# ZhenghaoFei/visual_odom

Hardware: AMD Instinct MI355X
Metric: stereo frames/sec on KITTI-00 1241x376 @ ~2000 features (higher is better)
Workload: dtype u8/int32 LK (f32 2x2 solve), f64 pose solve

## Files before the change

visual_odom_amd/csrc/lk.hip:

```cpp
#include "vo_kernels.h"
#include "vo_lkmath.h"

#include <float.h>

namespace vo {

constexpr int LK_WIN = 21;
constexpr int LK_JT_W = 48, LK_JT_H = 40;
constexpr int LK_W_BITS = 14;

struct __attribute__((packed, aligned(1))) LkU2 {
    uint32_t lo, hi;
};
struct __attribute__((packed, aligned(4))) LkU4 {
    uint32_t a, b, c, d;
};

__device__ __forceinline__ void lk_weights(float a, float b, uint32_t &wt, uint32_t &wb)
{
    const float s = (float)(1 << LK_W_BITS), magic = 12582912.f;
    const float a1 = (1.f - a) * s, a0 = a * s, b1 = 1.f - b;
    const uint32_t r00 = (uint32_t)__float_as_int(a1 * b1 + magic);
    const uint32_t r01 = (uint32_t)__float_as_int(a0 * b1 + magic);
    const uint32_t r10 = (uint32_t)__float_as_int(a1 * b + magic);
    const uint32_t iw11 = ((1u << LK_W_BITS) + 3u * 0x4B400000u) - (r00 + r01 + r10);
    wt = perm_b32(r01, r00, VO_SEL_LO16);
    wb = perm_b32(iw11, r10, VO_SEL_LO16);
}

#ifndef VO_LK_ATTRS
#define VO_LK_ATTRS __launch_bounds__(64, 7)
#endif
template <bool SPLIT>
__device__ __forceinline__ void lk_circular_body(const PyrImage *__restrict__ imgs, const Quad *__restrict__ quads,
                                                 const float2 *__restrict__ pts_in, const int *__restrict__ n_pts, int cap,
                                                 int n_frames, int fpg , int ppp ,
                                                 float2 *__restrict__ trk,
                                                 uint8_t *__restrict__ status,
                                                 const LkParams prm, int hop_begin, int hop_end)
{
    __shared__ __attribute__((aligned(16))) uint8_t s_jt[LK_JT_H * LK_JT_W];

    const int bid = blockIdx.x;
    const int xcd = bid & 7, slot = bid >> 3;
    const int grp = slot / ppp, fi = slot - grp * ppp;
    const int frame = grp * fpg + (xcd & (fpg - 1));
    const int f = (xcd / fpg) * ppp + fi;
    if (frame >= n_frames || f >= n_pts[frame])
        return;
    const int lane = threadIdx.x;
    const bool live = lane < 63;
    const int lr = live ? lane : 62;
    const int r = lr / 3, c0 = 7 * (lr - 3 * r);
    const int lane_off = r * LK_JT_W + c0;

    const Quad q = quads[frame];
    const float halfWin = (LK_WIN - 1) * 0.5f;
    const float FLT_SCALE = 1.f / (1 << 20);
    const float eps_lo = (float)(prm.epsilon * 0.999999), eps_hi = (float)(prm.epsilon * 1.000001);
    const float min_eig_n = prm.min_eig * (1.001f * (float)(2 * LK_WIN * LK_WIN));

    const float2 p = pts_in[(size_t)frame * cap + f];
    float prevPtX = unif(p.x), prevPtY = unif(p.y);
    if (SPLIT && hop_begin > 0) {
        const size_t o = ((size_t)frame * 4 + (hop_begin - 1)) * cap + f;
        const float2 q0 = trk[o];
        const bool dead0 = status[o] == 0 || q0.x < 0.f || q0.y < 0.f || (hop_begin == 1 && (p.x < 0.f || p.y < 0.f));
        if (dead0 && !prm.full_chain)
            return;
        prevPtX = unif(q0.x);
        prevPtY = unif(q0.y);
    }

    for (int hop = SPLIT ? hop_begin : 0; hop < (SPLIT ? hop_end : 4); hop++) {
        const int pi = hop == 0 ? q.l0 : hop == 1 ? q.r0 : hop == 2 ? q.r1 : q.l1;
        const int ni = hop == 0 ? q.r0 : hop == 1 ? q.r1 : hop == 2 ? q.l1 : q.l0;
        const PyrImage &I = imgs[pi];
        const PyrImage &J = imgs[ni];
        float outX = 0.f, outY = 0.f;
        int st = 1;

        for (int level = prm.max_level; level >= 0; level--) {
            const float scale = __int_as_float((127 - level) << 23);
            float prevX = prevPtX * scale, prevY = prevPtY * scale;
            float nextX, nextY;
            if (level == prm.max_level) {
                nextX = prevX;
                nextY = prevY;
            } else {
                nextX = outX * 2.f;
                nextY = outY * 2.f;
            }
            outX = nextX;
            outY = nextY;

            const int iw = I.w[level], ih = I.h[level], istride = I.stride[level];
            const int jw = J.w[level], jh = J.h[level], jstride = J.stride[level];
            const VO_GLOBAL uint8_t *__restrict__ Iimg = (const VO_GLOBAL uint8_t *)I.lvl[level];
            const VO_GLOBAL uint32_t *__restrict__ Ider = (const VO_GLOBAL uint32_t *)I.der[level];
            const VO_GLOBAL uint8_t *__restrict__ Jimg = (const VO_GLOBAL uint8_t *)J.lvl[level];

            prevX -= halfWin;
            prevY -= halfWin;
            const float fpx = floorf(prevX), fpy = floorf(prevY);
            const int ipx = uni(vo_f2i(fpx)), ipy = uni(vo_f2i(fpy));
            if (VO_BALLOT(__builtin_isunordered(fpx, fpy)) != 0ull || ipx < -LK_WIN || ipx >= iw || ipy < -LK_WIN || ipy >= ih) {
                if (level == 0)
                    st = 0;
                continue;
            }
            uint32_t wt, wb;
            lk_weights(prevX - fpx, prevY - fpy, wt, wb);

            uint32_t Ixp[4], Iyp[4];
            int a11 = 0, a12 = 0, a22 = 0, c1 = 0, c2 = 0;
            {
                const ptrdiff_t org = (ptrdiff_t)VO_BY * istride + VO_BX;
                const VO_GLOBAL uint8_t *Ib = Iimg - org;
                const VO_GLOBAL uint8_t *Db = (const VO_GLOBAL uint8_t *)(Ider - org);
                const uint32_t o = (uint32_t)((ipy + r + VO_BY) * istride + ipx + c0 + VO_BX);
                const uint32_t od = live ? 4u * o : 0u, drow = 4u * (uint32_t)istride;
                const LkU2 t = *(const VO_GLOBAL LkU2 *)(Ib + o);
                const LkU2 u = *(const VO_GLOBAL LkU2 *)(Ib + (o + (uint32_t)istride));
                const LkU4 dt0 = *(const VO_GLOBAL LkU4 *)(Db + od);
                const LkU4 dt1 = *(const VO_GLOBAL LkU4 *)(Db + (od + 16u));
                const LkU4 db0 = *(const VO_GLOBAL LkU4 *)(Db + (od + drow));
                const LkU4 db1 = *(const VO_GLOBAL LkU4 *)(Db + (od + drow + 16u));
                const uint32_t dt[8] = {dt0.a, dt0.b, dt0.c, dt0.d, dt1.a, dt1.b, dt1.c, dt1.d};
                const uint32_t db[8] = {db0.a, db0.b, db0.c, db0.d, db1.a, db1.b, db1.c, db1.d};
                uint32_t Ip[4];
                bilinear7_u8(t.lo, t.hi, u.lo, u.hi, wt, wb, Ip);
                bilinear7_deriv(dt, db, wt, wb, Ixp, Iyp);
                a11 = sdot2_first(Ixp[0], Ixp[0], 0);
                a12 = sdot2_first(Ixp[0], Iyp[0], 0);
                a22 = sdot2_first(Iyp[0], Iyp[0], 0);
                c1 = sdot2_first(Ip[0], Ixp[0], 0);
                c2 = sdot2_first(Ip[0], Iyp[0], 0);
#pragma unroll
                for (int m = 1; m < 4; m++) {
                    a11 = sdot2(Ixp[m], Ixp[m], a11);
                    a12 = sdot2(Ixp[m], Iyp[m], a12);
                    a22 = sdot2(Iyp[m], Iyp[m], a22);
                    c1 = sdot2(Ip[m], Ixp[m], c1);
                    c2 = sdot2(Ip[m], Iyp[m], c2);
                }
            }
            float A11, A12, A22;
            wave_sum3_exact_f32(a11, a12, a22, A11, A12, A22);
            A11 *= FLT_SCALE;
            A12 *= FLT_SCALE;
            A22 *= FLT_SCALE;

            float D = A11 * A22 - A12 * A12;
            const float t = A22 + A11;
            const float s2 = (A11 - A22) * (A11 - A22) + 4.f * A12 * A12;
            const float u = t - (min_eig_n + t * 3.814697265625e-6f);
            bool eig_ok = u > 0.f && s2 < u * u * 0.9999f;
            if (__builtin_expect(!eig_ok, 0)) {
#ifndef VO_HOST_EMUL
                asm volatile("" ::: "memory");
#endif
                const float minEig = (t - sqrtf(s2)) / (float)(2 * LK_WIN * LK_WIN);
                eig_ok = !(minEig < prm.min_eig);
            }
            if (!eig_ok || D < FLT_EPSILON) {
                if (level == 0)
                    st = 0;
                continue;
            }
            D = 1.f / D;
            const float A11s = A11 * FLT_SCALE, A12s = A12 * FLT_SCALE, A22s = A22 * FLT_SCALE;
            const int nc1 = -c1, nc2 = -c2;

            nextX -= halfWin;
            nextY -= halfWin;
            float prevDX = 0.f, prevDY = 0.f;
            int jx0 = 0, jy0 = 0;
            bool have_tile = false;
            static_assert(LK_JT_W % 16 == 0 && VO_BX % 4 == 0, "16-byte tile chunks at 4-byte aligned origins");
            static_assert(VO_BY >= LK_WIN && LK_JT_W >= LK_WIN + 1 + 12 + 3 && LK_JT_H >= LK_WIN + 1 + 9,
                          "a tile clamped to the row end / the last border row still covers the window of every corner the "
                          "reference admits (up to w - 1, h - 1: the borders are at least a window wide)");
            const int jx_max = jstride - VO_BX - LK_JT_W, jy_max = jh + VO_BY - LK_JT_H;

            int j = 0;
            float fnx = floorf(nextX), fny = floorf(nextY);
            bool run = prm.max_count > 0;
            while (run) {
                const int inx = uni(vo_f2i(fnx)), iny = uni(vo_f2i(fny));
                if (VO_BALLOT(__builtin_isunordered(fnx, fny)) != 0ull || inx < -LK_WIN || inx >= jw || iny < -LK_WIN || iny >= jh) {
                    if (level == 0)
                        st = 0;
                    break;
                }
                if (!have_tile || inx < jx0 || inx + LK_WIN + 1 > jx0 + LK_JT_W || iny < jy0 ||
                    iny + LK_WIN + 1 > jy0 + LK_JT_H) {
                    jx0 = (inx - 12) & ~3;
                    jy0 = iny - 9;
                    jx0 = jx0 < -VO_BX ? -VO_BX : jx0 > jx_max ? jx_max : jx0;
                    jy0 = jy0 < -VO_BY ? -VO_BY : jy0 > jy_max ? jy_max : jy0;
                    __syncthreads();
                    const VO_GLOBAL uint8_t *tb = Jimg + (ptrdiff_t)jy0 * jstride + jx0;
                    for (int c = lane; c < LK_JT_H * (LK_JT_W / 16); c += 64) {
                        const int row = c / (LK_JT_W / 16), col = c - row * (LK_JT_W / 16);
                        const LkU4 v = *(const VO_GLOBAL LkU4 *)(tb + (uint32_t)(row * jstride + 16 * col));
                        *reinterpret_cast<uint4 *>(&s_jt[row * LK_JT_W + 16 * col]) = make_uint4(v.a, v.b, v.c, v.d);
                    }
                    __syncthreads();
                    have_tile = true;
                }
                uint32_t Jt[7], Jb[7];
                {
                    const int off = (iny - jy0) * LK_JT_W + (inx - jx0) + lane_off;
                    const LkU2 t = *reinterpret_cast<const LkU2 *>(&s_jt[off]);
                    const LkU2 u = *reinterpret_cast<const LkU2 *>(&s_jt[off + LK_JT_W]);
                    lift7(t.lo, t.hi, Jt);
                    lift7(u.lo, u.hi, Jb);
                }
                for (;;) {
                    lk_weights(nextX - fnx, nextY - fny, wt, wb);
                    int b1, b2;
                    {
                        uint32_t Jp[4];
                        blend7(Jt, Jb, wt, wb, Jp);
                        b1 = sdot2_first(Jp[0], Ixp[0], nc1);
                        b2 = sdot2_first(Jp[0], Iyp[0], nc2);
#pragma unroll
                        for (int m = 1; m < 4; m++) {
                            b1 = sdot2(Jp[m], Ixp[m], b1);
                            b2 = sdot2(Jp[m], Iyp[m], b2);
                        }
                    }
                    float fb1, fb2;
                    wave_sum2_exact_f32(b1, b2, fb1, fb2);
                    const float dx = (A12s * fb2 - A22s * fb1) * D;
                    const float dy = (A12s * fb1 - A11s * fb2) * D;
                    nextX += dx;
                    nextY += dy;
                    outX = nextX + halfWin;
                    outY = nextY + halfWin;
                    const float n2 = fmaf(dy, dy, dx * dx);
                    if (__builtin_expect(!(n2 > eps_hi), 0)) {
#ifndef VO_HOST_EMUL
                        asm volatile("" ::: "memory");
#endif
                        if (n2 < eps_lo || (double)dx * dx + (double)dy * dy <= prm.epsilon) {
                            run = false;
                            break;
                        }
                    }
                    if (j > 0 && fabsf(dx + prevDX) <= 0.01f && fabsf(dy + prevDY) <= 0.01f) {
#ifndef VO_HOST_EMUL
                        asm volatile("" ::: "memory");
#endif
                        outX -= dx * 0.5f;
                        outY -= dy * 0.5f;
                        run = false;
                        break;
                    }
                    prevDX = dx;
                    prevDY = dy;
                    if (++j >= prm.max_count) {
                        run = false;
                        break;
                    }
                    const uint32_t ua = (uint32_t)__float_as_int(nextX - fnx), ub = (uint32_t)__float_as_int(nextY - fny);
                    if (VO_BALLOT((ua > ub ? ua : ub) >= 0x3f800000u) != 0ull) {
                        fnx = floorf(nextX);
                        fny = floorf(nextY);
                        break;
                    }
                }
            }

            if (st && level == 0) {
                const int fx = vo_f2i(floorf(outX - halfWin)), fy = vo_f2i(floorf(outY - halfWin));
                if (fx < -LK_WIN || fx >= jw || fy < -LK_WIN || fy >= jh)
                    st = 0;
            }
        }

        if (lane == 0) {
            trk[((size_t)frame * 4 + hop) * cap + f] = make_float2(outX, outY);
            status[((size_t)frame * 4 + hop) * cap + f] = (uint8_t)st;
        }
        const bool dead = st == 0 || outX < 0.f || outY < 0.f || (hop == 0 && (p.x < 0.f || p.y < 0.f));
        if (dead && !prm.full_chain && hop < 3) {
            if (lane == 0)
                for (int k = hop + 1; k < 4; k++) {
                    trk[((size_t)frame * 4 + k) * cap + f] = make_float2(-1.f, -1.f);
                    status[((size_t)frame * 4 + k) * cap + f] = 0;
                }
            return;
        }
        prevPtX = unif(outX);
        prevPtY = unif(outY);
    }
}

__global__ VO_LK_ATTRS void lk_circular_kernel(const PyrImage *__restrict__ imgs,
                                                          const Quad *__restrict__ quads,
                                                          const float2 *__restrict__ pts_in,
                                                          const int *__restrict__ n_pts, int cap,
                                                          int n_frames, int fpg ,
                                                          int ppp ,
                                                          float2 *__restrict__ trk,
                                                          uint8_t *__restrict__ status,
                                                          LkParams prm)
{
    lk_circular_body<false>(imgs, quads, pts_in, n_pts, cap, n_frames, fpg, ppp, trk, status, prm, 0, 4);
}

__global__ VO_LK_ATTRS void lk_hops_kernel(const PyrImage *__restrict__ imgs, const Quad *__restrict__ quads,
                                           const float2 *__restrict__ pts_in, const int *__restrict__ n_pts, int cap,
                                           int n_frames, int fpg, int ppp, float2 *__restrict__ trk,
                                           uint8_t *__restrict__ status, LkParams prm, int hop_begin, int hop_end)
{
    lk_circular_body<true>(imgs, quads, pts_in, n_pts, cap, n_frames, fpg, ppp, trk, status, prm, hop_begin, hop_end);
}

#if defined(VO_DEV_VARIANTS) || defined(VO_HOST_EMUL)
__device__ __forceinline__ void half_sum2_exact_f32(int a, int b, float &fa, float &fb)
{
    VO_PERMLANE16_SWAP(a, b);
    int t = a + b;
    t = dpp_add<VO_DPP_QUAD_XOR1, 0xf>(t);
    int hi = t >> 16, lo = t & 0xffff;
    hi = dpp_add<VO_DPP_QUAD_XOR2, 0xf>(hi);
    lo = dpp_add<VO_DPP_QUAD_XOR2, 0xf>(lo);
    hi = dpp_add<VO_DPP_ROW_HALF_MIRROR, 0xf>(hi);
    lo = dpp_add<VO_DPP_ROW_HALF_MIRROR, 0xf>(lo);
    hi = dpp_add<VO_DPP_ROW_MIRROR, 0xf>(hi);
    lo = dpp_add<VO_DPP_ROW_MIRROR, 0xf>(lo);
    const float res = fmaf((float)hi, 65536.f, (float)lo);
    int x = __float_as_int(res), y = x;
    VO_PERMLANE16_SWAP(x, y);
    fa = __int_as_float(x);
    fb = __int_as_float(y);
}

#ifndef VO_LK_PAIR_ATTRS
#define VO_LK_PAIR_ATTRS __launch_bounds__(64, 4)
#endif
__global__ VO_LK_PAIR_ATTRS void lk_circular_pair_kernel(const PyrImage *__restrict__ imgs,
                                                         const Quad *__restrict__ quads,
                                                         const float2 *__restrict__ pts_in,
                                                         const int *__restrict__ n_pts, int cap, int n_frames,
                                                         int fpg , int ppp ,
                                                         float2 *__restrict__ trk,
                                                         uint8_t *__restrict__ status,
                                                         LkParams prm)
{
    __shared__ __attribute__((aligned(16))) uint8_t s_jt[2 * LK_JT_H * LK_JT_W];

    const int bid = blockIdx.x;
    const int xcd = bid & 7, slot = bid >> 3;
    const int grp = slot / ppp, fi = slot - grp * ppp;
    const int frame = grp * fpg + (xcd & (fpg - 1));
    if (frame >= n_frames)
        return;
    const int lane = threadIdx.x, half = lane >> 5, hl = lane & 31;
    const int f = 2 * ((xcd / fpg) * ppp + fi) + half;
    bool act = f < n_pts[frame];
    if (VO_BALLOT(act) == 0ull)
        return;
    const int sA = 2 * hl, sB = 2 * hl + 1;
    const bool liveB = sB < 63;
    const int sBc = liveB ? sB : 62;
    const int rA = sA / 3, cA = 7 * (sA - 3 * rA), rB = sBc / 3, cB = 7 * (sBc - 3 * rB);
    const int offA = rA * LK_JT_W + cA, offB = rB * LK_JT_W + cB;
    uint8_t *const tile = s_jt + half * (LK_JT_H * LK_JT_W);

    const Quad q = quads[frame];
    const float halfWin = (LK_WIN - 1) * 0.5f;
    const float FLT_SCALE = 1.f / (1 << 20);
    const float eps_lo = (float)(prm.epsilon * 0.999999), eps_hi = (float)(prm.epsilon * 1.000001);
    const float min_eig_n = prm.min_eig * (1.001f * (float)(2 * LK_WIN * LK_WIN));

    float2 p = make_float2(0.f, 0.f);
    if (act)
        p = pts_in[(size_t)frame * cap + f];
    float prevPtX = p.x, prevPtY = p.y;

    for (int hop = 0; hop < 4; hop++) {
        const int pi = hop == 0 ? q.l0 : hop == 1 ? q.r0 : hop == 2 ? q.r1 : q.l1;
        const int ni = hop == 0 ? q.r0 : hop == 1 ? q.r1 : hop == 2 ? q.l1 : q.l0;
        const PyrImage &I = imgs[pi];
        const PyrImage &J = imgs[ni];
        float outX = 0.f, outY = 0.f;
        int st = 1;

        for (int level = prm.max_level; level >= 0; level--) {
            const float scale = __int_as_float((127 - level) << 23);
            float prevX = prevPtX * scale, prevY = prevPtY * scale;
            float nextX, nextY;
            if (level == prm.max_level) {
                nextX = prevX;
                nextY = prevY;
            } else {
                nextX = outX * 2.f;
                nextY = outY * 2.f;
            }
            outX = nextX;
            outY = nextY;

            const int iw = I.w[level], ih = I.h[level], istride = I.stride[level];
            const int jw = J.w[level], jh = J.h[level], jstride = J.stride[level];
            const VO_GLOBAL uint8_t *__restrict__ Iimg = (const VO_GLOBAL uint8_t *)I.lvl[level];
            const VO_GLOBAL uint32_t *__restrict__ Ider = (const VO_GLOBAL uint32_t *)I.der[level];
            const VO_GLOBAL uint8_t *__restrict__ Jimg = (const VO_GLOBAL uint8_t *)J.lvl[level];

            prevX -= halfWin;
            prevY -= halfWin;
            const float fpx = floorf(prevX), fpy = floorf(prevY);
            const int ipx = vo_f2i(fpx), ipy = vo_f2i(fpy);
            const bool in = act && !(__builtin_isunordered(fpx, fpy) || ipx < -LK_WIN || ipx >= iw || ipy < -LK_WIN || ipy >= ih);
            if (act && !in && level == 0)
                st = 0;
            if (VO_BALLOT(in) == 0ull)
                continue;
            uint32_t wt, wb;
            lk_weights(prevX - fpx, prevY - fpy, wt, wb);

            uint32_t IxA[4], IyA[4], IxB[4], IyB[4];
            int a11, a12, a22, c1, c2;
            {
                const int ipxs = in ? ipx : 0, ipys = in ? ipy : 0;
                const ptrdiff_t org = (ptrdiff_t)VO_BY * istride + VO_BX;
                const VO_GLOBAL uint8_t *Ib = Iimg - org;
                const VO_GLOBAL uint8_t *Db = (const VO_GLOBAL uint8_t *)(Ider - org);
                const uint32_t drow = 4u * (uint32_t)istride;
#define VO_LK_SLOT(r, c0, live, Ixp, Iyp, FIRST)                                                                       \
    {                                                                                                                  \
        const uint32_t o = (uint32_t)((ipys + (r) + VO_BY) * istride + ipxs + (c0) + VO_BX);                           \
        const uint32_t od = (live) ? 4u * o : 0u;                                                                      \
        const LkU2 t = *(const VO_GLOBAL LkU2 *)(Ib + o);                                                              \
        const LkU2 u = *(const VO_GLOBAL LkU2 *)(Ib + (o + (uint32_t)istride));                                        \
        const LkU4 dt0 = *(const VO_GLOBAL LkU4 *)(Db + od);                                                           \
        const LkU4 dt1 = *(const VO_GLOBAL LkU4 *)(Db + (od + 16u));                                                   \
        const LkU4 db0 = *(const VO_GLOBAL LkU4 *)(Db + (od + drow));                                                  \
        const LkU4 db1 = *(const VO_GLOBAL LkU4 *)(Db + (od + drow + 16u));                                            \
        const uint32_t dt[8] = {dt0.a, dt0.b, dt0.c, dt0.d, dt1.a, dt1.b, dt1.c, dt1.d};                               \
        const uint32_t db[8] = {db0.a, db0.b, db0.c, db0.d, db1.a, db1.b, db1.c, db1.d};                               \
        uint32_t Ip[4];                                                                                                \
        bilinear7_u8(t.lo, t.hi, u.lo, u.hi, wt, wb, Ip);                                                              \
        bilinear7_deriv(dt, db, wt, wb, Ixp, Iyp);                                                                     \
        _Pragma("unroll") for (int m = 0; m < 4; m++)                                                                  \
        {                                                                                                              \
            if ((FIRST) && m == 0) {                                                                                   \
                a11 = sdot2_first(Ixp[0], Ixp[0], 0);                                                                  \
                a12 = sdot2_first(Ixp[0], Iyp[0], 0);                                                                  \
                a22 = sdot2_first(Iyp[0], Iyp[0], 0);                                                                  \
                c1 = sdot2_first(Ip[0], Ixp[0], 0);                                                                    \
                c2 = sdot2_first(Ip[0], Iyp[0], 0);                                                                    \
            } else {                                                                                                   \
                a11 = sdot2(Ixp[m], Ixp[m], a11);                                                                      \
                a12 = sdot2(Ixp[m], Iyp[m], a12);                                                                      \
                a22 = sdot2(Iyp[m], Iyp[m], a22);                                                                      \
                c1 = sdot2(Ip[m], Ixp[m], c1);                                                                         \
                c2 = sdot2(Ip[m], Iyp[m], c2);                                                                         \
            }                                                                                                          \
        }                                                                                                              \
    }
                VO_LK_SLOT(rA, cA, true, IxA, IyA, true)
                VO_LK_SLOT(rB, cB, liveB, IxB, IyB, false)
#undef VO_LK_SLOT
            }
            float A11, A12, A22, unused;
            half_sum2_exact_f32(a11, a12, A11, A12);
            half_sum2_exact_f32(a22, 0, A22, unused);
            A11 *= FLT_SCALE;
            A12 *= FLT_SCALE;
            A22 *= FLT_SCALE;

            float D = A11 * A22 - A12 * A12;
            const float t = A22 + A11;
            const float s2 = (A11 - A22) * (A11 - A22) + 4.f * A12 * A12;
            const float u = t - (min_eig_n + t * 3.814697265625e-6f);
            bool eig_ok = u > 0.f && s2 < u * u * 0.9999f;
            if (VO_BALLOT(in && !eig_ok) != 0ull) {
                const float minEig = (t - sqrtf(s2)) / (float)(2 * LK_WIN * LK_WIN);
                eig_ok = eig_ok || !(minEig < prm.min_eig);
            }
            const bool ok = in && eig_ok && !(D < FLT_EPSILON);
            if (in && !ok && level == 0)
                st = 0;
            if (VO_BALLOT(ok) == 0ull)
                continue;
            D = 1.f / D;
            const float A11s = A11 * FLT_SCALE, A12s = A12 * FLT_SCALE, A22s = A22 * FLT_SCALE;
            const int nc1 = -c1, nc2 = -c2;

            nextX -= halfWin;
            nextY -= halfWin;
            float prevDX = 0.f, prevDY = 0.f;
            int jx0 = 0, jy0 = 0, offT = 0;
            bool have_tile = false;
            const int jx_max = jstride - VO_BX - LK_JT_W, jy_max = jh + VO_BY - LK_JT_H;

            int j = 0;
            float fnx = floorf(nextX), fny = floorf(nextY);
            bool run = ok && prm.max_count > 0;
            bool entry = run;
            uint32_t JtA[7], JbA[7], JtB[7], JbB[7];
            while (VO_BALLOT(run) != 0ull) {
                if (VO_BALLOT(entry) != 0ull) {
                    const int inx = vo_f2i(fnx), iny = vo_f2i(fny);
                    const bool oob = entry && (__builtin_isunordered(fnx, fny) || inx < -LK_WIN || inx >= jw || iny < -LK_WIN || iny >= jh);
                    if (oob) {
                        if (level == 0)
                            st = 0;
                        run = false;
                    }
                    const bool e2 = entry && !oob;
                    const bool need = e2 && (!have_tile || inx < jx0 || inx + LK_WIN + 1 > jx0 + LK_JT_W || iny < jy0 ||
                                             iny + LK_WIN + 1 > jy0 + LK_JT_H);
                    if (VO_BALLOT(need) != 0ull) {
                        if (need) {
                            jx0 = (inx - 12) & ~3;
                            jy0 = iny - 9;
                            jx0 = jx0 < -VO_BX ? -VO_BX : jx0 > jx_max ? jx_max : jx0;
                            jy0 = jy0 < -VO_BY ? -VO_BY : jy0 > jy_max ? jy_max : jy0;
                        }
                        __syncthreads();
                        if (need) {
                            const VO_GLOBAL uint8_t *tb = Jimg + ((ptrdiff_t)jy0 * jstride + jx0);
                            for (int c = hl; c < LK_JT_H * (LK_JT_W / 16); c += 32) {
                                const int row = c / (LK_JT_W / 16), col = c - row * (LK_JT_W / 16);
                                const LkU4 v = *(const VO_GLOBAL LkU4 *)(tb + (uint32_t)(row * jstride + 16 * col));
                                *reinterpret_cast<uint4 *>(&tile[row * LK_JT_W + 16 * col]) = make_uint4(v.a, v.b, v.c, v.d);
                            }
                            have_tile = true;
                        }
                        __syncthreads();
                    }
                    if (e2)
                        offT = (iny - jy0) * LK_JT_W + (inx - jx0);
                    {
                        const LkU2 tA = *reinterpret_cast<const LkU2 *>(&tile[offT + offA]);
                        const LkU2 uA = *reinterpret_cast<const LkU2 *>(&tile[offT + offA + LK_JT_W]);
                        const LkU2 tB = *reinterpret_cast<const LkU2 *>(&tile[offT + offB]);
                        const LkU2 uB = *reinterpret_cast<const LkU2 *>(&tile[offT + offB + LK_JT_W]);
                        lift7(tA.lo, tA.hi, JtA);
                        lift7(uA.lo, uA.hi, JbA);
                        lift7(tB.lo, tB.hi, JtB);
                        lift7(uB.lo, uB.hi, JbB);
                    }
                    entry = false;
                    if (VO_BALLOT(run) == 0ull)
                        break;
                }
                lk_weights(nextX - fnx, nextY - fny, wt, wb);
                int b1, b2;
                {
                    uint32_t Jp[4];
                    blend7(JtA, JbA, wt, wb, Jp);
                    b1 = sdot2_first(Jp[0], IxA[0], nc1);
                    b2 = sdot2_first(Jp[0], IyA[0], nc2);
#pragma unroll
                    for (int m = 1; m < 4; m++) {
                        b1 = sdot2(Jp[m], IxA[m], b1);
                        b2 = sdot2(Jp[m], IyA[m], b2);
                    }
                    blend7(JtB, JbB, wt, wb, Jp);
#pragma unroll
                    for (int m = 0; m < 4; m++) {
                        b1 = sdot2(Jp[m], IxB[m], b1);
                        b2 = sdot2(Jp[m], IyB[m], b2);
                    }
                }
                float fb1, fb2;
                half_sum2_exact_f32(b1, b2, fb1, fb2);
                const float dx = (A12s * fb2 - A22s * fb1) * D;
                const float dy = (A12s * fb1 - A11s * fb2) * D;
                if (run) {
                    nextX += dx;
                    nextY += dy;
                    outX = nextX + halfWin;
                    outY = nextY + halfWin;
                    const float n2 = fmaf(dy, dy, dx * dx);
                    bool stop = false;
                    if (!(n2 > eps_hi))
                        stop = n2 < eps_lo || (double)dx * dx + (double)dy * dy <= prm.epsilon;
                    if (!stop && j > 0 && fabsf(dx + prevDX) <= 0.01f && fabsf(dy + prevDY) <= 0.01f) {
                        outX -= dx * 0.5f;
                        outY -= dy * 0.5f;
                        stop = true;
                    }
                    prevDX = dx;
                    prevDY = dy;
                    if (stop)
                        run = false;
                }
                if (++j >= prm.max_count)
                    run = false;
                if (run) {
                    const uint32_t ua = (uint32_t)__float_as_int(nextX - fnx), ub = (uint32_t)__float_as_int(nextY - fny);
                    if ((ua > ub ? ua : ub) >= 0x3f800000u) {
                        fnx = floorf(nextX);
                        fny = floorf(nextY);
                        entry = true;
                    }
                }
            }

            if (ok && st && level == 0) {
                const int fx = vo_f2i(floorf(outX - halfWin)), fy = vo_f2i(floorf(outY - halfWin));
                if (fx < -LK_WIN || fx >= jw || fy < -LK_WIN || fy >= jh)
                    st = 0;
            }
        }

        if (act && hl == 0) {
            trk[((size_t)frame * 4 + hop) * cap + f] = make_float2(outX, outY);
            status[((size_t)frame * 4 + hop) * cap + f] = (uint8_t)st;
        }
        const bool dead = st == 0 || outX < 0.f || outY < 0.f || (hop == 0 && (p.x < 0.f || p.y < 0.f));
        if (act && dead && !prm.full_chain && hop < 3) {
            if (hl == 0)
                for (int k = hop + 1; k < 4; k++) {
                    trk[((size_t)frame * 4 + k) * cap + f] = make_float2(-1.f, -1.f);
                    status[((size_t)frame * 4 + k) * cap + f] = 0;
                }
            act = false;
        }
        if (VO_BALLOT(act) == 0ull)
            return;
        prevPtX = outX;
        prevPtY = outY;
    }
}

#endif
#ifndef VO_HOST_EMUL
void launch_lk_circular(const PyrImage *d_imgs, const Quad *d_quads, const float2 *d_pts, const int *d_npts,
                        int cap, int max_pts, int n_frames, float2 *d_trk, uint8_t *d_status,
                        const LkParams &prm, hipStream_t stream)
{
    if (max_pts <= 0 || n_frames <= 0)
        return;
    const int fpg = n_frames >= 8 ? 8 : n_frames >= 4 ? 4 : n_frames >= 2 ? 2 : 1;
    const int parts = 8 / fpg, ppp = (max_pts + parts - 1) / parts;
    const int groups = (n_frames + fpg - 1) / fpg;
    dim3 grid((unsigned)(8 * groups * ppp));
    hipLaunchKernelGGL(lk_circular_kernel, grid, dim3(64), 0, stream, d_imgs, d_quads, d_pts, d_npts, cap, n_frames,
                       fpg, ppp, d_trk, d_status, prm);
}

void launch_lk_hops(const PyrImage *d_imgs, const Quad *d_quads, const float2 *d_pts, const int *d_npts, int cap, int max_pts,
                    int n_frames, float2 *d_trk, uint8_t *d_status, const LkParams &prm, int hop_begin, int hop_end,
                    hipStream_t stream)
{
    if (max_pts <= 0 || n_frames <= 0 || hop_begin < 0 || hop_end > 4 || hop_begin >= hop_end)
        return;
    const int fpg = n_frames >= 8 ? 8 : n_frames >= 4 ? 4 : n_frames >= 2 ? 2 : 1;
    const int parts = 8 / fpg, ppp = (max_pts + parts - 1) / parts;
    const int groups = (n_frames + fpg - 1) / fpg;
    dim3 grid((unsigned)(8 * groups * ppp));
    hipLaunchKernelGGL(lk_hops_kernel, grid, dim3(64), 0, stream, d_imgs, d_quads, d_pts, d_npts, cap, n_frames, fpg, ppp,
                       d_trk, d_status, prm, hop_begin, hop_end);
}

#ifdef VO_DEV_VARIANTS
void launch_lk_circular_pair(const PyrImage *d_imgs, const Quad *d_quads, const float2 *d_pts, const int *d_npts,
                             int cap, int max_pts, int n_frames, float2 *d_trk, uint8_t *d_status,
                             const LkParams &prm, hipStream_t stream)
{
    if (max_pts <= 0 || n_frames <= 0)
        return;
    const int fpg = n_frames >= 8 ? 8 : n_frames >= 4 ? 4 : n_frames >= 2 ? 2 : 1;
    const int parts = 8 / fpg, pairs = (max_pts + 1) / 2, ppp = (pairs + parts - 1) / parts;
    const int groups = (n_frames + fpg - 1) / fpg;
    dim3 grid((unsigned)(8 * groups * ppp));
    hipLaunchKernelGGL(lk_circular_pair_kernel, grid, dim3(64), 0, stream, d_imgs, d_quads, d_pts, d_npts, cap, n_frames,
                       fpg, ppp, d_trk, d_status, prm);
}
#endif

#endif

}
```

Before: 22620.

## Add two-slot LK kernel interleaving two features per wave with persistent point lists

Adds a new circular LK kernel in which each 64-lane wave runs a state machine over two feature slots (lanes 0-31 and 32-63). Each slot walks a list of up to 8 points, and the two slots share one reduction (wave_sum4) per iteration. The intent is to raise lane utilisation and amortise the reductions and launch cost across more work per wave. It also reuses a shared-memory tile of the next image across iterations. The old kernel is kept and used for small workloads below a points threshold. The cost is a more complex control flow, extra registers, and lanes that idle when one slot finishes first.

Result: slower. 14390, median of 2 (-36.4%).

```diff
diff --git a/visual_odom_amd/csrc/lk.hip b/visual_odom_amd/csrc/lk.hip
--- a/visual_odom_amd/csrc/lk.hip
+++ b/visual_odom_amd/csrc/lk.hip
@@ -298,15 +298,15 @@
     }
 }
 
-__global__ VO_LK_ATTRS void lk_circular_kernel(const PyrImage *__restrict__ imgs,
-                                                          const Quad *__restrict__ quads,
-                                                          const float2 *__restrict__ pts_in,
-                                                          const int *__restrict__ n_pts, int cap,
-                                                          int n_frames, int fpg ,
-                                                          int ppp ,
-                                                          float2 *__restrict__ trk,
-                                                          uint8_t *__restrict__ status,
-                                                          LkParams prm)
+__global__ VO_LK_ATTRS void lk_circular_one_kernel(const PyrImage *__restrict__ imgs,
+                                                   const Quad *__restrict__ quads,
+                                                   const float2 *__restrict__ pts_in,
+                                                   const int *__restrict__ n_pts, int cap,
+                                                   int n_frames, int fpg ,
+                                                   int ppp ,
+                                                   float2 *__restrict__ trk,
+                                                   uint8_t *__restrict__ status,
+                                                   LkParams prm)
 {
     lk_circular_body<false>(imgs, quads, pts_in, n_pts, cap, n_frames, fpg, ppp, trk, status, prm, 0, 4);
 }
@@ -317,6 +317,415 @@
                                            uint8_t *__restrict__ status, LkParams prm, int hop_begin, int hop_end)
 {
     lk_circular_body<true>(imgs, quads, pts_in, n_pts, cap, n_frames, fpg, ppp, trk, status, prm, hop_begin, hop_end);
+}
+
+#ifndef VO_LK_LIST
+#define VO_LK_LIST 8
+#endif
+constexpr int LK_LIST = VO_LK_LIST;
+
+__device__ __forceinline__ void wave_sum4_exact_f32(int a1, int a2, int b1, int b2, float &f1, float &f2)
+{
+    VO_PERMLANE32_SWAP(a1, b1);
+    int t1 = a1 + b1;
+    VO_PERMLANE32_SWAP(a2, b2);
+    int t2 = a2 + b2;
+    VO_PERMLANE16_SWAP(t1, t2);
+    int u = t1 + t2;
+    u = dpp_add<VO_DPP_QUAD_XOR1, 0xf>(u);
+    int hi = u >> 16, lo = u & 0xffff;
+    hi = dpp_add<VO_DPP_QUAD_XOR2, 0xf>(hi);
+    lo = dpp_add<VO_DPP_QUAD_XOR2, 0xf>(lo);
+    hi = dpp_add<VO_DPP_ROW_HALF_MIRROR, 0xf>(hi);
+    lo = dpp_add<VO_DPP_ROW_HALF_MIRROR, 0xf>(lo);
+    hi = dpp_add<VO_DPP_ROW_MIRROR, 0xf>(hi);
+    lo = dpp_add<VO_DPP_ROW_MIRROR, 0xf>(lo);
+    const float res = fmaf((float)hi, 65536.f, (float)lo);
+    int x = __float_as_int(res), y = x;
+    VO_PERMLANE16_SWAP(x, y);
+    f1 = __int_as_float(x);
+    f2 = __int_as_float(y);
+}
+
+enum Lk2Phase { LK2_ITER, LK2_CELL, LK2_LEVEL_END, LK2_LEVEL, LK2_HOP, LK2_HOP_END, LK2_NEXT, LK2_DONE };
+
+struct Lk2Half {
+    float nextX, nextY, fnx, fny, prevDX, prevDY, A11s, A12s, A22s, D, outX, outY;
+    int j;
+};
+
+struct Lk2Slot {
+    int ph, f, hop, level, st, have_tile, jx0, jy0, pneg;
+    float prevPtX, prevPtY;
+};
+
+struct Lk2Ctx {
+    const PyrImage *imgs;
+    const float2 *pts;
+    float2 *trk;
+    uint8_t *status;
+    const int *quad;
+    int cap, frame, lane, r, c0, lane_off;
+    bool live;
+    float eps_lo, eps_hi, min_eig_n;
+};
+
+__device__ __forceinline__ float lk2_read(float v, int l) { return __int_as_float(VO_READLANE(__float_as_int(v), l)); }
+
+template <int S>
+__device__ __forceinline__ void lk2_advance(const Lk2Ctx &c, const LkParams &prm, Lk2Slot &sl, Lk2Half &h, int &next,
+                                            int fend, uint8_t *__restrict__ tile, uint32_t (&Ixp)[4], uint32_t (&Iyp)[4],
+                                            int &nc1, int &nc2, uint32_t (&Jt)[7], uint32_t (&Jb)[7])
+{
+    const bool mine = S ? c.lane >= 32 : c.lane < 32;
+    const int src = 32 * S;
+    const float halfWin = (LK_WIN - 1) * 0.5f;
+    const float FLT_SCALE = 1.f / (1 << 20);
+    for (;;) {
+        sl.ph = uni(sl.ph);
+        sl.hop = uni(sl.hop);
+        sl.level = uni(sl.level);
+        if (sl.ph == LK2_NEXT) {
+            if (next >= fend) {
+                sl.ph = LK2_DONE;
+                return;
+            }
+            sl.f = next++;
+            const float2 p = c.pts[(size_t)c.frame * c.cap + sl.f];
+            sl.prevPtX = unif(p.x);
+            sl.prevPtY = unif(p.y);
+            sl.pneg = sl.prevPtX < 0.f || sl.prevPtY < 0.f;
+            sl.hop = 0;
+            sl.ph = LK2_HOP;
+        }
+        if (sl.ph == LK2_HOP) {
+            sl.st = 1;
+            sl.level = prm.max_level;
+            h.outX = mine ? 0.f : h.outX;
+            h.outY = mine ? 0.f : h.outY;
+            sl.ph = LK2_LEVEL;
+        }
+        const int hop = sl.hop;
+        const int hn = (hop + 1) & 3, ni = c.quad[hn ^ (hn >> 1)];
+        if (sl.ph == LK2_HOP_END) {
+            const float outX = lk2_read(h.outX, src), outY = lk2_read(h.outY, src);
+            const size_t o = ((size_t)c.frame * 4 + hop) * c.cap + sl.f;
+            if (c.lane == 0) {
+                c.trk[o] = make_float2(outX, outY);
+                c.status[o] = (uint8_t)sl.st;
+            }
+            const bool dead = sl.st == 0 || outX < 0.f || outY < 0.f || (hop == 0 && sl.pneg);
+            if (dead && !prm.full_chain && hop < 3) {
+                if (c.lane == 0)
+                    for (int k = hop + 1; k < 4; k++) {
+                        c.trk[((size_t)c.frame * 4 + k) * c.cap + sl.f] = make_float2(-1.f, -1.f);
+                        c.status[((size_t)c.frame * 4 + k) * c.cap + sl.f] = 0;
+                    }
+                sl.ph = LK2_NEXT;
+                continue;
+            }
+            if (hop == 3) {
+                sl.ph = LK2_NEXT;
+                continue;
+            }
+            sl.hop = hop + 1;
+            sl.prevPtX = outX;
+            sl.prevPtY = outY;
+            sl.ph = LK2_HOP;
+            continue;
+        }
+        const int level = sl.level;
+        const PyrImage &J = c.imgs[ni];
+        if (sl.ph == LK2_LEVEL_END) {
+            if (sl.st && level == 0) {
+                const int jw = J.w[0], jh = J.h[0];
+                const float outX = lk2_read(h.outX, src), outY = lk2_read(h.outY, src);
+                const int fx = vo_f2i(floorf(outX - halfWin)), fy = vo_f2i(floorf(outY - halfWin));
+                if (fx < -LK_WIN || fx >= jw || fy < -LK_WIN || fy >= jh)
+                    sl.st = 0;
+            }
+            sl.level = level - 1;
+            sl.ph = LK2_LEVEL;
+            continue;
+        }
+        if (sl.ph == LK2_LEVEL) {
+            if (level < 0) {
+                sl.ph = LK2_HOP_END;
+                continue;
+            }
+            const int pi = c.quad[hop ^ (hop >> 1)];
+            const PyrImage &I = c.imgs[pi];
+            const float scale = __int_as_float((127 - level) << 23);
+            float prevX = sl.prevPtX * scale, prevY = sl.prevPtY * scale;
+            float nextX, nextY;
+            if (level == prm.max_level) {
+                nextX = prevX;
+                nextY = prevY;
+            } else {
+                nextX = lk2_read(h.outX, src) * 2.f;
+                nextY = lk2_read(h.outY, src) * 2.f;
+            }
+            h.outX = mine ? nextX : h.outX;
+            h.outY = mine ? nextY : h.outY;
+
+            const int iw = I.w[level], ih = I.h[level], istride = I.stride[level];
+            const VO_GLOBAL uint8_t *__restrict__ Iimg = (const VO_GLOBAL uint8_t *)I.lvl[level];
+            const VO_GLOBAL uint32_t *__restrict__ Ider = (const VO_GLOBAL uint32_t *)I.der[level];
+
+            prevX -= halfWin;
+            prevY -= halfWin;
+            const float fpx = floorf(prevX), fpy = floorf(prevY);
+            const int ipx = uni(vo_f2i(fpx)), ipy = uni(vo_f2i(fpy));
+            if (VO_BALLOT(__builtin_isunordered(fpx, fpy)) != 0ull || ipx < -LK_WIN || ipx >= iw || ipy < -LK_WIN || ipy >= ih) {
+                if (level == 0)
+                    sl.st = 0;
+                sl.level = level - 1;
+                continue;
+            }
+            uint32_t wt, wb;
+            lk_weights(prevX - fpx, prevY - fpy, wt, wb);
+            int a11, a12, a22, c1, c2;
+            {
+                const ptrdiff_t org = (ptrdiff_t)VO_BY * istride + VO_BX;
+                const VO_GLOBAL uint8_t *Ib = Iimg - org;
+                const VO_GLOBAL uint8_t *Db = (const VO_GLOBAL uint8_t *)(Ider - org);
+                const uint32_t o = (uint32_t)((ipy + c.r + VO_BY) * istride + ipx + c.c0 + VO_BX);
+                const uint32_t od = c.live ? 4u * o : 0u, drow = 4u * (uint32_t)istride;
+                const LkU2 t = *(const VO_GLOBAL LkU2 *)(Ib + o);
+                const LkU2 u = *(const VO_GLOBAL LkU2 *)(Ib + (o + (uint32_t)istride));
+                const LkU4 dt0 = *(const VO_GLOBAL LkU4 *)(Db + od);
+                const LkU4 dt1 = *(const VO_GLOBAL LkU4 *)(Db + (od + 16u));
+                const LkU4 db0 = *(const VO_GLOBAL LkU4 *)(Db + (od + drow));
+                const LkU4 db1 = *(const VO_GLOBAL LkU4 *)(Db + (od + drow + 16u));
+                const uint32_t dt[8] = {dt0.a, dt0.b, dt0.c, dt0.d, dt1.a, dt1.b, dt1.c, dt1.d};
+                const uint32_t db[8] = {db0.a, db0.b, db0.c, db0.d, db1.a, db1.b, db1.c, db1.d};
+                uint32_t Ip[4];
+                bilinear7_u8(t.lo, t.hi, u.lo, u.hi, wt, wb, Ip);
+                bilinear7_deriv(dt, db, wt, wb, Ixp, Iyp);
+                a11 = sdot2_first(Ixp[0], Ixp[0], 0);
+                a12 = sdot2_first(Ixp[0], Iyp[0], 0);
+                a22 = sdot2_first(Iyp[0], Iyp[0], 0);
+                c1 = sdot2_first(Ip[0], Ixp[0], 0);
+                c2 = sdot2_first(Ip[0], Iyp[0], 0);
+#pragma unroll
+                for (int m = 1; m < 4; m++) {
+                    a11 = sdot2(Ixp[m], Ixp[m], a11);
+                    a12 = sdot2(Ixp[m], Iyp[m], a12);
+                    a22 = sdot2(Iyp[m], Iyp[m], a22);
+                    c1 = sdot2(Ip[m], Ixp[m], c1);
+                    c2 = sdot2(Ip[m], Iyp[m], c2);
+                }
+            }
+            float A11, A12, A22;
+            wave_sum3_exact_f32(a11, a12, a22, A11, A12, A22);
+            A11 *= FLT_SCALE;
+            A12 *= FLT_SCALE;
+            A22 *= FLT_SCALE;
+            float D = A11 * A22 - A12 * A12;
+            const float t = A22 + A11;
+            const float s2 = (A11 - A22) * (A11 - A22) + 4.f * A12 * A12;
+            const float u = t - (c.min_eig_n + t * 3.814697265625e-6f);
+            bool eig_ok = u > 0.f && s2 < u * u * 0.9999f;
+            if (__builtin_expect(!eig_ok, 0)) {
+#ifndef VO_HOST_EMUL
+                asm volatile("" ::: "memory");
+#endif
+                const float minEig = (t - sqrtf(s2)) / (float)(2 * LK_WIN * LK_WIN);
+                eig_ok = !(minEig < prm.min_eig);
+            }
+            if (!eig_ok || D < FLT_EPSILON) {
+                if (level == 0)
+                    sl.st = 0;
+                sl.level = level - 1;
+                continue;
+            }
+            D = 1.f / D;
+            const float A11s = A11 * FLT_SCALE, A12s = A12 * FLT_SCALE, A22s = A22 * FLT_SCALE;
+            nc1 = -c1;
+            nc2 = -c2;
+            nextX -= halfWin;
+            nextY -= halfWin;
+            h.A11s = mine ? A11s : h.A11s;
+            h.A12s = mine ? A12s : h.A12s;
+            h.A22s = mine ? A22s : h.A22s;
+            h.D = mine ? D : h.D;
+            h.nextX = mine ? nextX : h.nextX;
+            h.nextY = mine ? nextY : h.nextY;
+            h.fnx = mine ? floorf(nextX) : h.fnx;
+            h.fny = mine ? floorf(nextY) : h.fny;
+            h.prevDX = mine ? 0.f : h.prevDX;
+            h.prevDY = mine ? 0.f : h.prevDY;
+            h.j = mine ? 0 : h.j;
+            sl.have_tile = 0;
+            sl.ph = prm.max_count > 0 ? LK2_CELL : LK2_LEVEL_END;
+            continue;
+        }
+        const int jw = J.w[level], jh = J.h[level], jstride = J.stride[level];
+        const float fnx = lk2_read(h.fnx, src), fny = lk2_read(h.fny, src);
+        const int inx = vo_f2i(fnx), iny = vo_f2i(fny);
+        if (VO_BALLOT(__builtin_isunordered(fnx, fny)) != 0ull || inx < -LK_WIN || inx >= jw || iny < -LK_WIN || iny >= jh) {
+            if (level == 0)
+                sl.st = 0;
+            sl.ph = LK2_LEVEL_END;
+            continue;
+        }
+        int jx0 = sl.jx0, jy0 = sl.jy0;
+        if (!sl.have_tile || inx < jx0 || inx + LK_WIN + 1 > jx0 + LK_JT_W || iny < jy0 || iny + LK_WIN + 1 > jy0 + LK_JT_H) {
+            const int jx_max = jstride - VO_BX - LK_JT_W, jy_max = jh + VO_BY - LK_JT_H;
+            jx0 = (inx - 12) & ~3;
+            jy0 = iny - 9;
+            jx0 = jx0 < -VO_BX ? -VO_BX : jx0 > jx_max ? jx_max : jx0;
+            jy0 = jy0 < -VO_BY ? -VO_BY : jy0 > jy_max ? jy_max : jy0;
+            __syncthreads();
+            const VO_GLOBAL uint8_t *tb = (const VO_GLOBAL uint8_t *)J.lvl[level] + ((ptrdiff_t)jy0 * jstride + jx0);
+            for (int k = c.lane; k < LK_JT_H * (LK_JT_W / 16); k += 64) {
+                const int row = k / (LK_JT_W / 16), col = k - row * (LK_JT_W / 16);
+                const LkU4 v = *(const VO_GLOBAL LkU4 *)(tb + (uint32_t)(row * jstride + 16 * col));
+                *reinterpret_cast<uint4 *>(&tile[row * LK_JT_W + 16 * col]) = make_uint4(v.a, v.b, v.c, v.d);
+            }
+            __syncthreads();
+            sl.have_tile = 1;
+            sl.jx0 = jx0;
+            sl.jy0 = jy0;
+        }
+        {
+            const int off = (iny - jy0) * LK_JT_W + (inx - jx0) + c.lane_off;
+            const LkU2 t = *reinterpret_cast<const LkU2 *>(&tile[off]);
+            const LkU2 u = *reinterpret_cast<const LkU2 *>(&tile[off + LK_JT_W]);
+            lift7(t.lo, t.hi, Jt);
+            lift7(u.lo, u.hi, Jb);
+        }
+        sl.ph = LK2_ITER;
+        return;
+    }
+}
+
+template <int S>
+__device__ __forceinline__ void lk2_residual(const uint32_t (&Jt)[7], const uint32_t (&Jb)[7], const uint32_t (&Ixp)[4],
+                                             const uint32_t (&Iyp)[4], int nc1, int nc2, uint32_t wt, uint32_t wb, int &b1,
+                                             int &b2)
+{
+    const uint32_t ws = (uint32_t)VO_READLANE((int)wt, 32 * S), wbs = (uint32_t)VO_READLANE((int)wb, 32 * S);
+    uint32_t Jp[4];
+    blend7(Jt, Jb, ws, wbs, Jp);
+    b1 = sdot2_first(Jp[0], Ixp[0], nc1);
+    b2 = sdot2_first(Jp[0], Iyp[0], nc2);
+#pragma unroll
+    for (int m = 1; m < 4; m++) {
+        b1 = sdot2(Jp[m], Ixp[m], b1);
+        b2 = sdot2(Jp[m], Iyp[m], b2);
+    }
+}
+
+#ifndef VO_LK2_ATTRS
+#define VO_LK2_ATTRS __launch_bounds__(64, 4)
+#endif
+__global__ VO_LK2_ATTRS void lk_circular_kernel(const PyrImage *__restrict__ imgs,
+                                                const Quad *__restrict__ quads,
+                                                const float2 *__restrict__ pts_in,
+                                                const int *__restrict__ n_pts, int cap,
+                                                int n_frames, int fpg ,
+                                                int ppp ,
+                                                float2 *__restrict__ trk,
+                                                uint8_t *__restrict__ status,
+                                                LkParams prm)
+{
+    __shared__ __attribute__((aligned(16))) uint8_t s_jt[2 * LK_JT_H * LK_JT_W];
+
+    if (ppp <= 0)
+        return;
+    const int bid = blockIdx.x;
+    const int xcd = bid & 7, wl = bid >> 3;
+    const int nl = (ppp + LK_LIST - 1) / LK_LIST;
+    const int grp = wl / nl, li = wl - grp * nl;
+    const int frame = grp * fpg + (xcd & (fpg - 1));
+    if (frame >= n_frames)
+        return;
+    const int part0 = (xcd / fpg) * ppp, npf = n_pts[frame];
+    const int lend = part0 + (li * LK_LIST + LK_LIST < ppp ? li * LK_LIST + LK_LIST : ppp);
+    const int fend = lend < npf ? lend : npf;
+    int next = part0 + li * LK_LIST;
+    if (next >= fend)
+        return;
+
+    Lk2Ctx c;
+    c.imgs = imgs;
+    c.pts = pts_in;
+    c.trk = trk;
+    c.status = status;
+    c.quad = (const int *)(quads + frame);
+    c.cap = cap;
+    c.frame = frame;
+    c.lane = threadIdx.x;
+    c.live = c.lane < 63;
+    const int lr = c.live ? c.lane : 62;
+    c.r = lr / 3;
+    c.c0 = 7 * (lr - 3 * c.r);
+    c.lane_off = c.r * LK_JT_W + c.c0;
+    c.eps_lo = (float)(prm.epsilon * 0.999999);
+    c.eps_hi = (float)(prm.epsilon * 1.000001);
+    c.min_eig_n = prm.min_eig * (1.001f * (float)(2 * LK_WIN * LK_WIN));
+    const float halfWin = (LK_WIN - 1) * 0.5f;
+
+    Lk2Slot sa, sb;
+    sa.ph = sb.ph = LK2_NEXT;
+    sa.have_tile = sb.have_tile = 0;
+    sa.jx0 = sa.jy0 = sb.jx0 = sb.jy0 = 0;
+    Lk2Half h = {0.f, 0.f, 0.f, 0.f, 0.f, 0.f, 0.f, 0.f, 0.f, 0.f, 0.f, 0.f, 0};
+    uint32_t IxA[4], IyA[4], IxB[4], IyB[4], JtA[7], JbA[7], JtB[7], JbB[7];
+    int nc1A = 0, nc2A = 0, nc1B = 0, nc2B = 0;
+
+    for (;;) {
+        if (sa.ph != LK2_ITER && sa.ph != LK2_DONE)
+            lk2_advance<0>(c, prm, sa, h, next, fend, s_jt, IxA, IyA, nc1A, nc2A, JtA, JbA);
+        if (sb.ph != LK2_ITER && sb.ph != LK2_DONE)
+            lk2_advance<1>(c, prm, sb, h, next, fend, s_jt + LK_JT_H * LK_JT_W, IxB, IyB, nc1B, nc2B, JtB, JbB);
+        const bool itA = sa.ph == LK2_ITER, itB = sb.ph == LK2_ITER;
+        if (!itA && !itB)
+            return;
+        uint32_t wt, wb;
+        lk_weights(h.nextX - h.fnx, h.nextY - h.fny, wt, wb);
+        int b1A = 0, b2A = 0, b1B = 0, b2B = 0;
+        if (itA)
+            lk2_residual<0>(JtA, JbA, IxA, IyA, nc1A, nc2A, wt, wb, b1A, b2A);
+        if (itB)
+            lk2_residual<1>(JtB, JbB, IxB, IyB, nc1B, nc2B, wt, wb, b1B, b2B);
+        float fb1, fb2;
+        wave_sum4_exact_f32(b1A, b2A, b1B, b2B, fb1, fb2);
+        const float dx = (h.A12s * fb2 - h.A22s * fb1) * h.D;
+        const float dy = (h.A12s * fb1 - h.A11s * fb2) * h.D;
+        h.nextX += dx;
+        h.nextY += dy;
+        h.outX = h.nextX + halfWin;
+        h.outY = h.nextY + halfWin;
+        const float n2 = fmaf(dy, dy, dx * dx);
+        bool stop = false;
+        if (__builtin_expect(!(n2 > c.eps_hi), 0))
+            stop = n2 < c.eps_lo || (double)dx * dx + (double)dy * dy <= prm.epsilon;
+        if (!stop && h.j > 0 && fabsf(dx + h.prevDX) <= 0.01f && fabsf(dy + h.prevDY) <= 0.01f) {
+            h.outX -= dx * 0.5f;
+            h.outY -= dy * 0.5f;
+            stop = true;
+        }
+        h.prevDX = dx;
+        h.prevDY = dy;
+        if (++h.j >= prm.max_count)
+            stop = true;
+        bool left = false;
+        if (!stop) {
+            const uint32_t ua = (uint32_t)__float_as_int(h.nextX - h.fnx), ub = (uint32_t)__float_as_int(h.nextY - h.fny);
+            if ((ua > ub ? ua : ub) >= 0x3f800000u) {
+                h.fnx = floorf(h.nextX);
+                h.fny = floorf(h.nextY);
+                left = true;
+            }
+        }
+        const uint64_t ms = VO_BALLOT(stop), ml = VO_BALLOT(left);
+        if (itA)
+            sa.ph = (ms & 1ull) ? LK2_LEVEL_END : (ml & 1ull) ? LK2_CELL : LK2_ITER;
+        if (itB)
+            sb.ph = ((ms >> 32) & 1ull) ? LK2_LEVEL_END : ((ml >> 32) & 1ull) ? LK2_CELL : LK2_ITER;
+    }
 }
 
 #if defined(VO_DEV_VARIANTS) || defined(VO_HOST_EMUL)
@@ -633,6 +1042,9 @@
 
 #endif
 #ifndef VO_HOST_EMUL
+#ifndef VO_LK_TWO_SLOT_MIN_POINTS
+#define VO_LK_TWO_SLOT_MIN_POINTS 32768
+#endif
 void launch_lk_circular(const PyrImage *d_imgs, const Quad *d_quads, const float2 *d_pts, const int *d_npts,
                         int cap, int max_pts, int n_frames, float2 *d_trk, uint8_t *d_status,
                         const LkParams &prm, hipStream_t stream)
@@ -642,9 +1054,15 @@
     const int fpg = n_frames >= 8 ? 8 : n_frames >= 4 ? 4 : n_frames >= 2 ? 2 : 1;
     const int parts = 8 / fpg, ppp = (max_pts + parts - 1) / parts;
     const int groups = (n_frames + fpg - 1) / fpg;
-    dim3 grid((unsigned)(8 * groups * ppp));
-    hipLaunchKernelGGL(lk_circular_kernel, grid, dim3(64), 0, stream, d_imgs, d_quads, d_pts, d_npts, cap, n_frames,
-                       fpg, ppp, d_trk, d_status, prm);
+    if ((long long)n_frames * max_pts >= VO_LK_TWO_SLOT_MIN_POINTS) {
+        dim3 grid((unsigned)(8 * groups * ((ppp + LK_LIST - 1) / LK_LIST)));
+        hipLaunchKernelGGL(lk_circular_kernel, grid, dim3(64), 0, stream, d_imgs, d_quads, d_pts, d_npts, cap, n_frames,
+                           fpg, ppp, d_trk, d_status, prm);
+    } else {
+        dim3 grid((unsigned)(8 * groups * ppp));
+        hipLaunchKernelGGL(lk_circular_one_kernel, grid, dim3(64), 0, stream, d_imgs, d_quads, d_pts, d_npts, cap, n_frames,
+                           fpg, ppp, d_trk, d_status, prm);
+    }
 }
 
 void launch_lk_hops(const PyrImage *d_imgs, const Quad *d_quads, const float2 *d_pts, const int *d_npts, int cap, int max_pts,
```
